# eltoto1219/vltk

Measured on AMD Instinct MI355X. Metric: images/sec FRCNN feature extraction, 800x1333 batch, higher is better.
Workload: dtype f16; 1 GPU; configs[1]: ResNet-101-C4 fp16 (the reference has no FPN: SURVEY.md D1), 32 synthetic 800x1333 images per GPU per step, R=300 RPN proposals through the Res5 head, max 100 detections/img, seeded synthetic weights; global_batch=32, parallelism=image-sharded x1, all-gather of output blocks

## Files before the change

include/vltk_hip.h:

```cpp
#ifndef VLTK_HIP_H
#define VLTK_HIP_H

#include <stddef.h>
#include <stdint.h>

#ifdef __cplusplus
extern "C" {
#endif

#define VK_OK 0
#define VK_EINVAL 1
#define VK_ENOTIMPL 2
#define VK_ENONFINITE 3
#define VK_EWEIGHTS 4
#define VK_EHIP 5
#define VK_ENOMEM 6

typedef enum { VK_F32 = 0, VK_F16 = 1, VK_I64 = 2, VK_I32 = 3, VK_BF16 = 4 } vk_dtype;
typedef enum { VK_ACT_NONE = 0, VK_ACT_RELU = 1, VK_ACT_GELU = 2 , VK_ACT_TANH = 3 } vk_act;

#define VK_MAX_ANCHOR_DIM 8
#define VK_MAX_NMS_THRESH 8

typedef struct vk_config {
// ... 130 lines not shown
int vk_memcpy_d2d(void *dst_dev, const void *src_dev, size_t bytes, void *stream);

int vk_enable_stage_timing(vk_handle *h, int enable);
int vk_get_stage_timing(vk_handle *h, float *ms6);

#define VK_NUM_KERNEL_BUCKETS 12
int vk_enable_kernel_timing(vk_handle *h, int enable);
int vk_get_kernel_timing(vk_handle *h, int64_t *launches, double *ms, double *flops, double *bytes, int reset);


size_t vk_packed_weight_bytes(int cout, int cin, int kh, int kw, int groups, vk_dtype dt);
int vk_packed_cout(int cout);
int vk_conv_slice_channels(int cin, int groups);
int vk_pack_conv_weight(const float *w_oihw_host, const float *bn_host, const float *bias_host,
                        int cout, int cin, int kh, int kw, int groups, vk_dtype dt,
                        void *w_packed_host, float *bias_packed_host);

int vk_conv2d(const void *x, int N, int H, int W, int cin,
              const void *w_packed, const float *bias_packed, const void *residual,
              void *y, int cout, int ldy, int kh, int kw, int stride, int pad, int dil, int groups,
              int relu, vk_dtype dt, vk_dtype out_dt, void *stream);

#define VK_ROUTE_GENERIC 0
#define VK_ROUTE_RING 1
#define VK_ROUTE_DUO 2
#define VK_ROUTE_WS 3
#define VK_ROUTE_GEMM4 4
#define VK_ROUTE_PANEL 5
#define VK_ROUTE_BLK 6
int vk_conv_route(int N, int H, int W, int cin, int cin2, int has_residual, int fused_mean, int cout, int ldy, int kh, int kw,
                  int stride, int pad, int dil, int groups, int relu, vk_dtype dt, vk_dtype out_dt);
int vk_panel_phase_images(int N, int H, int W, int dil);
int vk_panel_phase_tile_rows(int N, int H, int W, int dil, int cout);

int vk_conv1x1_dual(const void *x1, int cin1, const void *x2, int cin2, long M,
                    const void *w_packed, const float *bias_packed, const void *residual,
                    void *y, int cout, int relu, void *stream);

int vk_bottleneck64(const void *x, int N, int H, int W, int cin, int proj,
                    const void *w1_packed, const float *b1_packed, const void *w2_packed, const float *b2_packed,
                    const void *w3_packed, const float *b3_packed, void *y, void *stream);

int vk_fuse_shortcut(int cin, int cin_shortcut, int cout, int stride, vk_dtype dt);
int vk_bottleneck64_eligible(int cin, int cmid, int cout, int stride, int dil, int groups, int proj, int fused_shortcut,
                             long N, int H, int W, vk_dtype dt);

size_t vk_conv1x1_meanpool_workspace_bytes(int N, int HW, int cout);
int vk_conv1x1_meanpool(const void *x, int N, int HW, int cin, const void *w_packed, const float *bias_packed,
                        const void *residual, int cout, int relu, float *out_mean,
                        void *workspace, size_t workspace_bytes, void *stream);


int vk_linear(const void *x, long M, int K, const void *w_packed, const float *bias_packed, const void *residual,
              void *y, int N, int ldy, int act, vk_dtype dt, vk_dtype out_dt, void *stream);
int vk_layernorm(const void *x, int ldx, const float *gamma, const float *beta, void *y, int ldy, int M, int C,
                 float eps, float scale, int accumulate, vk_dtype dt, void *stream);
int vk_embed_layernorm(const int64_t *input_ids, const int64_t *token_type_ids, int B, int L, const void *word,
                       const void *position, const void *token_type, const float *gamma, const float *beta,
                       void *y, int C, float eps, vk_dtype dt, void *stream);
int vk_attention(const void *q, int ldq, const void *k, int ldk, const void *v, int ldv, const float *mask,
                 void *out, int ldo, int B, int heads, int Lq, int Lk, int d, vk_dtype dt, void *stream);
int vk_attention_tiled(const void *q, int ldq, const void *k, int ldk, const void *v, int ldv, const float *mask,
                       void *out, int ldo, int B, int heads, int Lq, int Lk, int d, vk_dtype dt, void *stream);
#define VK_ATT_ROUTE_MFMA 0
#define VK_ATT_ROUTE_LDS 1
#define VK_ATT_ROUTE_TILED 2
// ... 132 lines not shown
```

vltk_amd/_lib.py:

```python
import ctypes as C
import os

_HERE = os.path.dirname(os.path.abspath(__file__))
LIB_PATH = os.path.join(_HERE, "libvltk_hip.so")
if os.environ.get("VLTK_AMD_LIB"):
    LIB_PATH = os.environ["VLTK_AMD_LIB"]
elif os.environ.get("VLTK_AMD_ABLATION_LIB") == "1":
    LIB_PATH = LIB_PATH.replace("libvltk_hip.so", "libvltk_hip_ablation.so")

VK_OK, VK_EINVAL, VK_ENOTIMPL, VK_ENONFINITE, VK_EWEIGHTS, VK_EHIP, VK_ENOMEM = range(7)
VK_F32, VK_F16, VK_I64, VK_I32, VK_BF16 = 0, 1, 2, 3, 4
VK_ACT_NONE, VK_ACT_RELU, VK_ACT_GELU, VK_ACT_TANH = 0, 1, 2, 3
VK_ROUTE_GENERIC, VK_ROUTE_RING, VK_ROUTE_DUO, VK_ROUTE_WS, VK_ROUTE_GEMM4, VK_ROUTE_PANEL, VK_ROUTE_BLK = range(7)
VK_ATT_ROUTE_MFMA, VK_ATT_ROUTE_LDS, VK_ATT_ROUTE_TILED, VK_ATT_ROUTE_STREAM = range(4)
VK_MAX_ANCHOR_DIM = 8
VK_MAX_NMS_THRESH = 8
VK_MAX_IGNOREY = 64
VK_SELECT_CLASS_MAX, VK_SELECT_PER_CLASS, VK_SELECT_DETECTIONS = 0, 1, 2
VK_POOLER_ROIPOOL, VK_POOLER_ROIALIGN, VK_POOLER_ROIALIGNV2 = 0, 1, 2

_EXC = {
    VK_EINVAL: ValueError,
    VK_ENOTIMPL: NotImplementedError,
    VK_ENONFINITE: AssertionError,
# ... 58 lines not shown
    "vk_option_check": (_I, [C.c_char_p, _I]),
    "vk_option_default": (_I, [C.c_char_p, C.POINTER(_I)]),
    "vk_pooler_check": (_I, [_I, _I]),
    "vk_set_pooler": (_I, [_P, _I, _I]),
    "vk_get_pooler": (_I, [_P, C.POINTER(_I), C.POINTER(_I)]),
    "vk_num_weights": (_I, [_P, C.POINTER(_I)]),
    "vk_weight_name": (_I, [_P, _I, C.POINTER(C.c_char_p)]),
    "vk_forward": (_I, [_P, _P, _I, _I, _I, _P, _P, C.POINTER(vk_roi_params), C.POINTER(vk_outputs), _P]),
    "vk_forward_begin": (_I, [_P, _P, _I, _I, _I, _P, _P, C.POINTER(vk_roi_params), C.POINTER(vk_outputs), _P,
                              C.POINTER(C.c_int64)]),
    "vk_forward_begin_ignorey": (_I, [_P, _P, _I, _I, _I, _P, _P, C.POINTER(vk_roi_params), C.POINTER(vk_outputs), _P,
                                      C.POINTER(C.c_int64), C.POINTER(vk_ignorey)]),
    "vk_forward_begin_select": (_I, [_P, _P, _I, _I, _I, _P, _P, C.POINTER(vk_select_params), C.POINTER(vk_outputs), _P,
                                     C.POINTER(C.c_int64), C.POINTER(vk_ignorey)]),
    "vk_forward_boxes_begin": (_I, [_P, _P, _I, _I, _I, _P, _P, _P, _I, _P, C.POINTER(vk_outputs), _P, C.POINTER(C.c_int64)]),
    "vk_forward_grid_begin": (_I, [_P, _P, _I, _I, _I, _P, _P, _I, _I, C.POINTER(vk_outputs), _P, C.POINTER(C.c_int64)]),
    "vk_grid_pool": (_I, [_P, _I, _I, _I, _I, _I, _P, _P, _I, _I, _I, _P, _I, _P, _P]),
    "vk_forward_end": (_I, [_P, C.c_int64]),
    "vk_given_boxes_ingest": (_I, [_P, _P, _P, _P, _I, _I, _P, _P, _P, _I, _I, _F, _I, _P, _P]),
    "vk_given_box_outputs": (_I, [_P, _P, _P, _P, _P, _P, _P, _P, _I, _I, _I, C.POINTER(vk_outputs), _P]),
    "vk_get_stage": (_I, [_P, C.c_char_p, C.POINTER(_P), C.POINTER(_I), C.POINTER(C.c_int64), C.POINTER(_I)]),
    "vk_memcpy_d2d": (_I, [_P, _P, _SZ, _P]),
    "vk_enable_stage_timing": (_I, [_P, _I]),
    "vk_get_stage_timing": (_I, [_P, C.POINTER(_F)]),
    "vk_enable_kernel_timing": (_I, [_P, _I]),
    "vk_get_kernel_timing": (_I, [_P, C.POINTER(C.c_int64), C.POINTER(_D), C.POINTER(_D), C.POINTER(_D), _I]),
    "vk_packed_weight_bytes": (_SZ, [_I, _I, _I, _I, _I, _I]),
    "vk_conv_slice_channels": (_I, [_I, _I]),
    "vk_packed_cout": (_I, [_I]),
    "vk_pack_conv_weight": (_I, [_P, _P, _P, _I, _I, _I, _I, _I, _I, _P, _P]),
    "vk_conv_route": (_I, [_I] * 18),
    "vk_panel_phase_images": (_I, [_I, _I, _I, _I]),
    "vk_panel_phase_tile_rows": (_I, [_I, _I, _I, _I, _I]),
    "vk_conv1x1_dual": (_I, [_P, _I, _P, _I, C.c_long, _P, _P, _P, _P, _I, _I, _P]),
    "vk_bottleneck64": (_I, [_P, _I, _I, _I, _I, _I, _P, _P, _P, _P, _P, _P, _P, _P]),
    "vk_fuse_shortcut": (_I, [_I, _I, _I, _I, _I]),
    "vk_bottleneck64_eligible": (_I, [_I, _I, _I, _I, _I, _I, _I, _I, C.c_long, _I, _I, _I]),
    "vk_conv1x1_meanpool_workspace_bytes": (_SZ, [_I, _I, _I]),
    "vk_conv1x1_meanpool": (_I, [_P, _I, _I, _I, _P, _P, _P, _I, _I, _P, _P, _SZ, _P]),
    "vk_linear": (_I, [_P, C.c_long, _I, _P, _P, _P, _P, _I, _I, _I, _I, _I, _P]),
    "vk_layernorm": (_I, [_P, _I, _P, _P, _P, _I, _I, _I, _F, _F, _I, _I, _P]),
    "vk_embed_layernorm": (_I, [_P, _P, _I, _I, _P, _P, _P, _P, _P, _P, _I, _F, _I, _P]),
    "vk_attention": (_I, [_P, _I, _P, _I, _P, _I, _P, _P, _I, _I, _I, _I, _I, _I, _I, _P]),
    "vk_attention_tiled": (_I, [_P, _I, _P, _I, _P, _I, _P, _P, _I, _I, _I, _I, _I, _I, _I, _P]),
    "vk_attention_route": (_I, [_I] * 9),
    "vk_visualbert_embed": (_I, [_P, _P, _P, _P, _I, _I, _I, _I, _P, _I, _P, _I, _P, _P, _I, _P, _P, _I, _P, _P, _P, _I, _F, _I, _P]),
    "vk_vit_patchify": (_I, [_P, _I, _I, _I, _I, _I, _P, _I, _I, _P]),
    "vk_vit_assemble": (_I, [_P, _I, _P, _P, _I, _I, _P, _I, _I, _P]),
    "vk_roi_align": (_I, [_P, _P, _P, _P, _I, _I, _I, _P, _P, _I, _I, _I, _I, _P, _I, _P]),
    "vk_assign_levels": (_I, [_P, _I, _I, _I, _I, _F, _I, _P, _P]),
    "vk_upsample2x_add": (_I, [_P, _P, _P, _I, _I, _I, _I, _I, _I, _I, _P]),
    "vk_subsample2": (_I, [_P, _P, _I, _I, _I, _I, _I, _P]),
    "vk_relu_copy": (_I, [_P, _P, C.c_long, _I, _P]),
    "vk_rpn_multilevel_workspace_bytes": (_SZ, [_I, _I, _I, _I]),
    "vk_rpn_proposals_multilevel": (_I, [_P, _P, _P, _P, _I, _I, _P, _P, _I, _P, _P, _F, _P, _P, _F, _D, _I, _I, _P, _P, _P, _P, _P, _SZ, _P]),
    "vk_rpn_proposals_multilevel_ignorey": (_I, [_P, _P, _P, _P, _I, _I, _P, _P, _I, _P, _P, _F, _P, _P, _F, _D, _I, _I, _P, _P, _P, _P,
                                                 _P, _SZ, _P, C.POINTER(vk_ignorey)]),
    "vk_conv2d": (_I, [_P, _I, _I, _I, _I, _P, _P, _P, _P, _I, _I, _I, _I, _I, _I, _I, _I, _I, _I, _I, _P]),
    "vk_nchw_to_nhwc": (_I, [_P, _I, _I, _I, _I, _P, _I, _P]),
    "vk_nhwc_to_nchw": (_I, [_P, _I, _I, _I, _I, _P, _I, _P]),
    "vk_packed_stem_bytes": (_SZ, [_I, _I]),
    "vk_pack_stem_weight": (_I, [_P, _P, _I, _I, _P, _P]),
    "vk_stem": (_I, [_P, _I, _I, _I, _P, _P, _I, _I, _P, _I, _P, _SZ, _P]),
    "vk_stem_workspace_bytes": (_SZ, [_I, _I, _I, _I, _I]),
    "vk_stem_out_hw": (None, [_I, _I, _I, C.POINTER(_I), C.POINTER(_I)]),
    "vk_preprocess": (_I, [_P, _P, _P, _I, _I, _I, C.POINTER(_F), C.POINTER(_F), _F, _P, _P]),
# ... 59 lines not shown
```

vltk_amd/csrc/conv3x3_panel.hip:

```cpp
#include <cstdio>
#include <type_traits>
#include <vector>

#include "vk_common.h"

namespace vk {

typedef _Float16 half8 __attribute__((ext_vector_type(8)));
typedef float floatx4 __attribute__((ext_vector_type(4)));
typedef _Float16 half4 __attribute__((ext_vector_type(4)));
typedef unsigned uintx4 __attribute__((ext_vector_type(4)));

struct PanelK {
    const char *x;
    const char *w;
    const float *bias;
    const char *res;
    char *y;
    int H, W, HW, M;
    int cin_bytes, ldy;
    int dil;
    int cstages;
    int wrow_bytes;
    int relu;
// ... 28 lines not shown
constexpr int panel_in_window() {
    int c = 0;
    for (int d = 1; d <= P_NW - 2; ++d) {
        int t = ((J - d) % 9 + 9) % 9;
        if (t < PP) ++c;
    }
    return c;
}
template <int J, int PP, int NWP, bool FIRST>
constexpr int pieces_in_window() {
    static_assert(PP <= 6, "a panel piece of the previous stage in the window of a tap other than 0");
    if (FIRST) return NWP * (P_NW - 2);
    const int c = NWP * (P_NW - 2) + panel_in_window<J, PP>();
    const int after_panel = NWP * (9 - PP);
    return J == 8 && after_panel < c ? after_panel : c;
}
template <int J, int PP, int NWP>
constexpr int last_in_window() {
    int c = 0;
    for (int d = 1; d <= P_NW - 2; ++d) {
        int t = J - d;
        if (t < 0 || t + P_NW < 9) c += NWP;
        if (t < 0 && 9 + t < PP) ++c;
    }
    return c;
}

template <int N>
__device__ __forceinline__ void vm_wait() {
    static_assert(N >= 0 && N <= 15, "vmcnt immediate");
    asm volatile("s_waitcnt vmcnt(%0)" ::"n"(N) : "memory");
}

template <int PP, int DBG, int TAG = 0, int MI = 8, int PHASE = 0, int WR = 2>
__global__ __launch_bounds__(512, 2) void conv3x3_panel_kernel(PanelK p) {
    extern __shared__ __attribute__((aligned(16))) char smem[];
    static_assert(MI == 8 || MI == 9, "8 or 9 row tiles per wave");
    static_assert(WR == 2 || WR == 4, "2 x 4 or 4 x 2 waves");
    static_assert(!PHASE || (PP == (WR == 4 ? 6 : 4) && MI == 8 && !(DBG & 9)), "the phase form: halo 128 = (W / 2 + 1) * 16 at W = 14, 256- or 512-row tiles");
    static_assert(WR == 2 || PHASE == 2, "512 x 128 tiles: the phase form only (a plain res4 launch would read its panel twice)");
    static_assert(MI == 8 || !(DBG & 8), "the LDS-staged epilogue is written for 128-row halves");
    constexpr int WC = 8 / WR;
    constexpr int CT = 64 * WC;
    constexpr int NWP = CT / 128;
    constexpr int WSLOT = CT * 64;
    constexpr int TILE = WR * MI * 16;
    constexpr int PROWS = PP * 128;
    constexpr int HALO = (PROWS - TILE) / 2;
    constexpr int PBYTES = PROWS * 64;
    constexpr int WBASE = 2 * PBYTES;
    static_assert(HALO >= (PHASE ? 128 : 48) && WBASE + P_NW * WSLOT + (PP == 3 || WR == 4 ? 256 : 0) <= 160 * 1024, "halo / LDS");
    constexpr bool ZROW = PP == 3;
    constexpr int ZOFF = WBASE + P_NW * WSLOT;

    int bid = blockIdx.x;
    const int nwg = p.m_tiles * p.n_tiles;
    unsigned long st_k0 = 0;
    if constexpr (DBG & 4) asm volatile("s_memrealtime %0\n\ts_waitcnt lgkmcnt(0)" : "=s"(st_k0)::"memory");
    if constexpr (PP == 3 || PHASE) {
        if (p.tile_ctr && bid >= p.static_tiles) {
            constexpr bool MAIL_IN_PANEL = PHASE && WR == 2;
            int *mail = reinterpret_cast<int *>(smem + (MAIL_IN_PANEL ? 0 : ZOFF + 128));
            if (threadIdx.x == 0) {
                const unsigned v = atomicAdd(p.tile_ctr, 1u);
                if (v == p.ctr_last) *p.tile_ctr = 0u;
                *mail = p.static_tiles + (int)v;
            }
            __syncthreads();
            bid = __builtin_amdgcn_readfirstlane(*mail);
            if constexpr (MAIL_IN_PANEL) __syncthreads();
            if (bid >= nwg) return;
        }
    }
    const int q = nwg >> 3, r = nwg & 7, xcd = bid & 7;
    const int t_ = (xcd < r ? xcd * (q + 1) : r * (q + 1) + (xcd - r) * q) + (bid >> 3);
    const int n_tile = t_ % p.n_tiles, m_tile = t_ / p.n_tiles;
    const int m0 = m_tile * TILE, n0 = n_tile * CT;

    const int tid = threadIdx.x, lane = tid & 63;
    const int wave = __builtin_amdgcn_readfirstlane(tid >> 6);
    const int wr = wave / WC, wc = wave & (WC - 1);
    const int g = lane >> 4, j = lane & 15;

// ... 50 lines not shown
    auto req_w = [&](int slot, int cs, int tap, int i) {
        const unsigned koff = (unsigned)(tap * p.cstages + cs) * 64;
        unsigned wb_ = wsrc0;
        asm volatile("" : "+v"(wb_));
        VKP_GLDS16(p.w + (wb_ + i * wstep + koff), smem + WBASE + slot * WSLOT + (wave * NWP + i) * 1024);
    };

    const unsigned lds0 = (unsigned)(unsigned long)(__attribute__((address_space(3))) char *)smem;
    [[maybe_unused]] const unsigned zrow = lds0 + ZOFF;
    if constexpr (ZROW) {
        if (tid < 16) *reinterpret_cast<unsigned *>(smem + ZOFF + tid * 4) = 0u;
        asm volatile("s_waitcnt lgkmcnt(0)" ::: "memory");
    }
    unsigned w_a[2];
#pragma unroll
    for (int par = 0; par < 2; ++par) {
        const int wrow = wc * 64 + (j >> 2) * 8 + par * 4 + (j & 3);
        w_a[par] = lds0 + WBASE + wrow * 64 + ((g ^ ((-(wrow >> 2)) & 3)) << 4);
    }
    const int jbase = HALO + wr * (MI * 16) + j;
    auto x_addr_of = [&](int parity, int tap) -> unsigned {
        const int shift = PHASE ? ((tap / 3 - 1) * (p.W >> 1) + (tap % 3 - 1)) * 16 : ((tap / 3 - 1) * p.W + (tap % 3 - 1)) * p.dil;
        int jb = jbase;
        asm volatile("" : "+v"(jb));
        const int rb = jb + shift;
        return lds0 + parity * PBYTES + (rb << 6) + ((g ^ ((-(rb >> 2)) & 3)) << 4);
    };

    floatx4 acc[MI][4];
#pragma unroll
    for (int mi = 0; mi < MI; ++mi)
#pragma unroll
        for (int ni = 0; ni < 4; ++ni) acc[mi][ni] = floatx4{0.f, 0.f, 0.f, 0.f};
    half8 wa[4], wb[4], xw[MI == 9 ? 5 : 4];
    const int CS = p.cstages;

#define VKP_DSR(dst, addr, OFF) asm volatile("ds_read_b128 %0, %1 offset:" #OFF : "=v"(dst) : "v"(addr))
#define VKP_DSRX(dst, addr, OFF, TW, J_, MI_)                                                        \
    do {                                                                                             \
        if constexpr (ZROW && !(DBG & 1)) {                                                          \
            unsigned m_, ad_;                                                                        \
            const unsigned zc_ = zrow - (OFF);                                                       \
            asm volatile("v_bfe_i32 %0, %1, %2, 1" : "=v"(m_) : "v"(TW), "n"(((J_) % 3) * 9 + (MI_))); \
            asm volatile("v_bfi_b32 %0, %1, %2, %3" : "=v"(ad_) : "v"(m_), "v"(addr), "s"(zc_));    \
            VKP_DSR(dst, ad_, OFF);                                                                  \
        } else                                                                                       \
            VKP_DSR(dst, addr, OFF);                                                                 \
    } while (0)
#define VKP_WAIT3(reg) asm volatile("s_waitcnt lgkmcnt(3)" : "+v"(reg))
#define VKP_WAIT4(reg) asm volatile("s_waitcnt lgkmcnt(4)" : "+v"(reg))
#define VKP_SB() __builtin_amdgcn_sched_barrier(0)
#define VKP_MMA_ROW(MI, XR, WF, TM)                                                                  \
    do {                                                                                             \
        if constexpr (PHASE == 2) {                                                                  \
            if (((TM) >> (MI)) & 1u) {                           \
                __builtin_amdgcn_s_setprio(1);                                                       \
                _Pragma("unroll") for (int ni = 0; ni < 4; ++ni) acc[MI][ni] =                       \
                    __builtin_amdgcn_mfma_f32_16x16x32_f16(WF[ni], XR, acc[MI][ni], 0, 0, 0);        \
                __builtin_amdgcn_s_setprio(0);                                                       \
            }                                                                                        \
            break;                                                                                   \
        }                                                                                            \
        if constexpr (!(DBG & 1) && !ZROW) {                                                         \
            uintx4 u_ = __builtin_bit_cast(uintx4, XR);                                              \
            const bool v_ = ((TM) >> (MI)) & 1u;                                                     \
            u_[0] = v_ ? u_[0] : 0u;                                                                 \
            u_[1] = v_ ? u_[1] : 0u;                                                                 \
// ... 10 lines not shown
    do {                                                \
        unsigned a0_ = w_a[0], a1_ = w_a[1];            \
        asm volatile("" : "+v"(a0_), "+v"(a1_));        \
        a0_ += so;                                      \
        a1_ += so;                                      \
        VKP_DSR(WF[0], a0_, 0);                         \
        VKP_DSR(WF[1], a1_, 0);                         \
        VKP_DSR(WF[2], a0_, 2048);                      \
        VKP_DSR(WF[3], a1_, 2048);                      \
    } while (0)

    auto tap_mask = [&](auto j_c) -> unsigned {
        constexpr int J = decltype(j_c)::value;
        unsigned tw = J < 3 ? vm0 : (J < 6 ? vm1 : vm2);
        if constexpr (PHASE)
            asm volatile("" : "+s"(tw));
        else
            asm volatile("" : "+v"(tw));
        return tw >> ((J % 3) * 9);
    };
    auto tap_word = [&](auto j_c) -> unsigned {
        constexpr int J = decltype(j_c)::value;
        unsigned tw = J < 3 ? vm0 : (J < 6 ? vm1 : vm2);
        asm volatile("" : "+v"(tw));
        return tw;
    };
    auto pre = [&](auto last_c, auto odd_c, auto j_c, unsigned xa, unsigned &xa_next, const half8 (&wcur)[4], auto first_c) {
        constexpr bool LAST = decltype(last_c)::value, FIRST = decltype(first_c)::value;
        constexpr int ODD = decltype(odd_c)::value;
        constexpr int J = decltype(j_c)::value;
        const unsigned tm = ZROW ? 0u : tap_mask(j_c);
        [[maybe_unused]] const unsigned tw = ZROW ? tap_word(j_c) : 0u;
        constexpr bool has_next = !(LAST && J == 8);
        if constexpr (has_next) xa_next = (J == 8) ? x_addr_of(1 - ODD, 0) : x_addr_of(ODD, J + 1);
        VKP_DSRX(xw[3], xa, 3072, tw, J, 3); VKP_WAIT3(xw[0]); VKP_SB(); VKP_MMA_ROW(0, xw[0], wcur, tm); VKP_SB();
        VKP_DSRX(xw[0], xa, 4096, tw, J, 4); VKP_WAIT3(xw[1]); VKP_SB(); VKP_MMA_ROW(1, xw[1], wcur, tm); VKP_SB();
        VKP_DSRX(xw[1], xa, 5120, tw, J, 5); VKP_WAIT3(xw[2]); VKP_SB(); VKP_MMA_ROW(2, xw[2], wcur, tm); VKP_SB();
        VKP_DSRX(xw[2], xa, 6144, tw, J, 6); VKP_WAIT3(xw[3]); VKP_SB(); VKP_MMA_ROW(3, xw[3], wcur, tm); VKP_SB();
        if constexpr (MI == 9) {
            VKP_DSRX(xw[3], xa, 7168, tw, J, 7); VKP_DSRX(xw[4], xa, 8192, tw, J, 8); VKP_WAIT4(xw[0]); VKP_SB(); VKP_MMA_ROW(4, xw[0], wcur, tm); VKP_SB();
            asm volatile("s_waitcnt lgkmcnt(0)" : "+v"(xw[1]), "+v"(xw[2]), "+v"(xw[3]), "+v"(xw[MI == 9 ? 4 : 3])::"memory");
        } else {
            VKP_DSRX(xw[3], xa, 7168, tw, J, 7); VKP_WAIT3(xw[0]); VKP_SB(); VKP_MMA_ROW(4, xw[0], wcur, tm); VKP_SB();
            asm volatile("s_waitcnt lgkmcnt(0)" : "+v"(xw[1]), "+v"(xw[2]), "+v"(xw[3])::"memory");
        }
        VKP_SB();
        if constexpr (has_next) {
            constexpr int OUT = LAST ? last_in_window<J, PP, NWP>() : pieces_in_window<J, PP, NWP, FIRST>();
            vm_wait<OUT>();
            if constexpr (!(DBG & 48) || ((DBG & 16) && J % 3 == 2)) asm volatile("s_barrier" ::: "memory");
        }
        VKP_SB();
    };
    auto post = [&](auto last_c, auto odd_c, auto j_c, int cs, unsigned xa_next, const half8 (&wcur)[4], half8 (&wnext)[4]) {
        constexpr bool LAST = decltype(last_c)::value;
        constexpr int ODD = decltype(odd_c)::value;
        constexpr int J = decltype(j_c)::value;
        static_assert(!(LAST && J == 8), "the final step has no POST");
        constexpr int SLOT = (3 * ODD + J) % P_NW;
        const unsigned tm = ZROW ? 0u : tap_mask(j_c);
        constexpr int JN = (J + 1) % 9;
        [[maybe_unused]] const unsigned twn = ZROW ? tap_word(std::integral_constant<int, JN>{}) : 0u;
        constexpr bool issue_w = !LAST || (J + P_NW < 9);
        constexpr bool issue_p = !LAST && (J < PP);
        constexpr unsigned so = (unsigned)((SLOT + 1) % P_NW) * WSLOT;
        VKP_READ_W(wnext, so);
        VKP_DSRX(xw[0], xa_next, 0, twn, JN, 0);
        VKP_SB();
        VKP_MMA_ROW(5, xw[1], wcur, tm);
        VKP_SB();
        if constexpr (issue_p) req_panel(cs + 1, J);
        if constexpr (issue_w) req_w(SLOT, cs + (J + P_NW) / 9, (J + P_NW) % 9, 0);
        VKP_DSRX(xw[1], xa_next, 1024, twn, JN, 1);
        VKP_SB();
        VKP_MMA_ROW(6, xw[2], wcur, tm);
        VKP_SB();
        if constexpr (issue_w && NWP == 2) req_w(SLOT, cs + (J + P_NW) / 9, (J + P_NW) % 9, 1);
        VKP_DSRX(xw[2], xa_next, 2048, twn, JN, 2);
        VKP_SB();
        VKP_MMA_ROW(7, xw[3], wcur, tm);
        VKP_SB();
        if constexpr (MI == 9) {
            VKP_MMA_ROW(8, xw[MI == 9 ? 4 : 3], wcur, tm);
            VKP_SB();
        }
    };
    auto wset = [&](auto u_c) -> half8(&)[4] {
        if constexpr (decltype(u_c)::value % 2 == 0)
            return wa;
        else
            return wb;
    };
#define VKP_IC(V) std::integral_constant<int, (V)> {}
#define VKP_UNIT(LP, LC, U)                                                                                          \
    post(LP, VKP_IC(((U) - 1) / 9), VKP_IC(((U) - 1) % 9), cs + ((U) - 1) / 9, xan, wset(VKP_IC((U) - 1)), wset(VKP_IC(U)));  \
    xa = xan;                                                                                                        \
    pre(LC, VKP_IC((U) / 9), VKP_IC((U) % 9), xa, xan, wset(VKP_IC(U)), F_{});
    using T_ = std::integral_constant<bool, true>;
    using F_ = std::integral_constant<bool, false>;

#pragma unroll
    for (int q2 = 0; q2 < PP; ++q2) req_panel(0, q2);
#pragma unroll
    for (int st = 0; st < P_NW; ++st) {
        req_w(st, 0, st, 0);
        if constexpr (NWP == 2) req_w(st, 0, st, 1);
    }
    if constexpr (PHASE) {
        unsigned u0 = 0, u1 = 0, u2 = 0;
#pragma unroll
        for (int mi = 0; mi < MI; ++mi) {
            int G;
            const PhaseBlk b = phase_blk(p, blk_of(wr * MI + mi, G));
// ... 52 lines not shown
            }
        }
    }

    vm_wait<NWP * (P_NW - 1)>();
    asm volatile("s_barrier" ::: "memory");
    unsigned long st_c0 = 0, st_r0 = 0;
    if constexpr (DBG & 4) asm volatile("s_memtime %0\n\ts_memrealtime %1\n\ts_waitcnt lgkmcnt(0)" : "=s"(st_c0), "=s"(st_r0)::"memory");
    unsigned xa = x_addr_of(0, 0), xan = 0;
    VKP_READ_W(wa, 0u);
    {
        [[maybe_unused]] const unsigned tw0 = tap_word(VKP_IC(0));
        VKP_DSRX(xw[0], xa, 0, tw0, 0, 0);
        VKP_DSRX(xw[1], xa, 1024, tw0, 0, 1);
        VKP_DSRX(xw[2], xa, 2048, tw0, 0, 2);
    }
    pre(F_{}, VKP_IC(0), VKP_IC(0), xa, xan, wa, T_{});
    int cs = 0;
    for (; cs + 2 < CS; cs += 2) {
        VKP_UNIT(F_{}, F_{}, 1) VKP_UNIT(F_{}, F_{}, 2) VKP_UNIT(F_{}, F_{}, 3) VKP_UNIT(F_{}, F_{}, 4) VKP_UNIT(F_{}, F_{}, 5)
        VKP_UNIT(F_{}, F_{}, 6) VKP_UNIT(F_{}, F_{}, 7) VKP_UNIT(F_{}, F_{}, 8) VKP_UNIT(F_{}, F_{}, 9) VKP_UNIT(F_{}, F_{}, 10)
        VKP_UNIT(F_{}, F_{}, 11) VKP_UNIT(F_{}, F_{}, 12) VKP_UNIT(F_{}, F_{}, 13) VKP_UNIT(F_{}, F_{}, 14) VKP_UNIT(F_{}, F_{}, 15)
        VKP_UNIT(F_{}, F_{}, 16) VKP_UNIT(F_{}, F_{}, 17)
        post(F_{}, VKP_IC(1), VKP_IC(8), cs + 1, xan, wb, wa);
        xa = xan;
        pre(F_{}, VKP_IC(0), VKP_IC(0), xa, xan, wa, F_{});
    }
    VKP_UNIT(F_{}, F_{}, 1) VKP_UNIT(F_{}, F_{}, 2) VKP_UNIT(F_{}, F_{}, 3) VKP_UNIT(F_{}, F_{}, 4) VKP_UNIT(F_{}, F_{}, 5)
    VKP_UNIT(F_{}, F_{}, 6) VKP_UNIT(F_{}, F_{}, 7) VKP_UNIT(F_{}, F_{}, 8) VKP_UNIT(F_{}, T_{}, 9) VKP_UNIT(T_{}, T_{}, 10)
    VKP_UNIT(T_{}, T_{}, 11) VKP_UNIT(T_{}, T_{}, 12) VKP_UNIT(T_{}, T_{}, 13) VKP_UNIT(T_{}, T_{}, 14) VKP_UNIT(T_{}, T_{}, 15)
    VKP_UNIT(T_{}, T_{}, 16) VKP_UNIT(T_{}, T_{}, 17)
    {
        const unsigned tm = ZROW ? 0u : tap_mask(VKP_IC(8));
        VKP_MMA_ROW(5, xw[1], wb, tm);
        VKP_MMA_ROW(6, xw[2], wb, tm);
        VKP_MMA_ROW(7, xw[3], wb, tm);
        if constexpr (MI == 9) VKP_MMA_ROW(8, xw[MI == 9 ? 4 : 3], wb, tm);
    }
    unsigned long st_c1 = 0, st_r1 = 0;
    if constexpr (DBG & 4) asm volatile("s_memtime %0\n\ts_memrealtime %1\n\ts_waitcnt lgkmcnt(0)" : "=s"(st_c1), "=s"(st_r1)::"memory");
#undef VKP_UNIT
#undef VKP_IC
#undef VKP_DSR
#undef VKP_DSRX
#undef VKP_WAIT3
#undef VKP_WAIT4
#undef VKP_MMA_ROW
#undef VKP_READ_W
#undef VKP_SB

    if constexpr (!(DBG & 8)) {
        if constexpr (PHASE) asm volatile("" : "+s"(g0), "+s"(gb0));
        auto epilogue = [&](auto res_c, auto relu_c, auto full_c) {
            constexpr bool RES = decltype(res_c)::value, RELU = decltype(relu_c)::value, FULL = decltype(full_c)::value;
            const int ch0 = n0 + wc * 64 + g * 8;
            floatx4 bq[2][2];
#pragma unroll
            for (int qn = 0; qn < 2; ++qn) {
                bq[qn][0] = *reinterpret_cast<const floatx4 *>(p.bias + ch0 + qn * 32);
                bq[qn][1] = *reinterpret_cast<const floatx4 *>(p.bias + ch0 + qn * 32 + 4);
            }
#pragma unroll
            for (int mi = 0; mi < MI; ++mi) {
                const long m = m0 + wr * (MI * 16) + mi * 16 + j;
                long mo = m;
                if constexpr (PHASE) {
                    int G;
                    const int t = blk_of(wr * MI + mi, G);
                    mo = (long)(G * 16 + j) * p.HW + phase_blk(p, t).row;
// ... 125 lines not shown
    if (panel_pp(a, 9) == 0) return 8;
    if (const char *v = getenv("VK_PANEL_MI")) {
        if (v[0] == '8') return 8;
        if (v[0] == '9') return 9;
    }
    const long nt = a.Cout / 256;
    const long n8 = ((M + 255) / 256 * nt + n_cu - 1) / n_cu, n9 = ((M + 287) / 288 * nt + n_cu - 1) / n_cu;
    if (n8 > 4) return 9;
    return n9 * 9 < n8 * 8 ? 9 : 8;
}

bool conv3x3_panel_eligible(const ConvArgs &a) {
    const char *v = getenv("VK_CONV3X3_PANEL");
    if (v && v[0] == '0') return false;
    if (a.stem || a.dt != VK_F16 || a.out_dt != VK_F16 || a.relu > 1) return false;
    if (a.kh != 3 || a.kw != 3 || a.stride != 1 || a.pad != a.dil) return false;
    if (a.Cout % 256 != 0 || a.ldy != a.Cout || a.Cin % 64 != 0 || a.Cin < 128) return false;
    if (panel_pp(a) == 0) return false;
    if ((long)a.N * a.H * a.W * a.Cin * 2 >= (1L << 32)) return false;
    return true;
}

int conv3x3_panel_phase_images(const ConvArgs &a) {
    const char *v = getenv("VK_PANEL_PHASE");
    if (v && v[0] == '0') return 0;
    if (a.dil != 2 || a.H % 2 != 0 || a.W % 2 != 0 || a.W > 14 || a.H > 1024 || a.N < 16) return 0;
    return a.N / 16 * 16;
}

int conv3x3_panel_phase_tile_rows(const ConvArgs &a) {
    if (a.Cout % 256 != 0 || conv3x3_panel_phase_images(a) == 0) return 0;
    const char *v = getenv("VK_PANEL_TALL");
    return v && v[0] == '0' ? 256 : 512;
}

static int launch_panel_one(const ConvArgs &a, hipStream_t stream, bool phase);

int launch_conv3x3_panel(const ConvArgs &a, hipStream_t stream) {
    const int np = conv3x3_panel_phase_images(a);
    if (np == 0) return launch_panel_one(a, stream, false);
    ConvArgs b = a;
    b.N = np;
    VK_TRY(launch_panel_one(b, stream, true));
    if (np == a.N) return VK_OK;
    const size_t rows = (size_t)np * a.H * a.W;
    b.N = a.N - np;
    b.x = (const char *)a.x + rows * a.Cin * 2;
    b.y = (char *)a.y + rows * a.ldy * 2;
    if (a.res) b.res = (const char *)a.res + rows * a.ldy * 2;
    return launch_panel_one(b, stream, false);
}

static int launch_panel_one(const ConvArgs &a, hipStream_t stream, bool phase) {
    DeviceState *ds = nullptr;
    VK_TRY(device_state(&ds));
    PanelK k;
    k.x = (const char *)a.x;
    k.w = (const char *)a.w;
    k.bias = a.bias;
    k.res = (const char *)a.res;
    k.y = (char *)a.y;
    k.H = a.H;
    k.W = a.W;
    k.HW = a.H * a.W;
    const long M = (long)a.N * a.H * a.W;
    VK_REQUIRE(M > 0 && M < (1L << 31) - 512, VK_EINVAL, "conv3x3_panel: M=%ld out of range", M);
// ... 49 lines not shown
        if (mi == 9)
            VKP_LAUNCH(3, 4, 0, 9);
        else
            VKP_LAUNCH(3, 4, 0, 8);
        VK_CHECK_HIP(hipStreamSynchronize(stream));
        std::vector<unsigned long> h((size_t)grid.x * 6);
        VK_CHECK_HIP(hipMemcpy(h.data(), k.stamps, nb, hipMemcpyDeviceToHost));
        VK_CHECK_HIP(hipFree(k.stamps));
        if (FILE *f = fopen(sf, "a")) {
            fprintf(f, "# wg k_loop_cycles k_loop_ticks workgroup_ticks ticks_before_k_loop start_tick end_tick (tick = 10 ns)\n");
            for (unsigned w = 0; w < grid.x; ++w)
                fprintf(f, "%u %lu %lu %lu %lu %lu %lu\n", w, h[(size_t)w * 6], h[(size_t)w * 6 + 1], h[(size_t)w * 6 + 2], h[(size_t)w * 6 + 3], h[(size_t)w * 6 + 4],
                        h[(size_t)w * 6 + 5]);
            fclose(f);
        }
    } else if (mi == 8 && pp == 3 && dbg == 8)
        VKP_LAUNCH(3, 8, 0, 8);
    else if (mi == 8 && pp == 3 && dbg == 1)
        VKP_LAUNCH(3, 1, 0, 8);
    else if (mi == 9 && pp == 3 && dbg == 1)
        VKP_LAUNCH(3, 1, 0, 9);
    else if (mi == 9 && pp == 3 && dbg == 16)
        VKP_LAUNCH(3, 16, 0, 9);
    else if (mi == 9 && pp == 3 && dbg == 32)
        VKP_LAUNCH(3, 32, 0, 9);
    else
#endif
#ifdef VK_ABLATION
    if (const char *pv = getenv("VK_PANEL_PHASE"); phase && pv && pv[0] == 'A') {
        VK_TRY(set_max_lds(conv3x3_panel_kernel<4, 0, 0, 8, 1>, smem));
        hipLaunchKernelGGL((conv3x3_panel_kernel<4, 0, 0, 8, 1>), grid, block, smem, stream, k);
    } else
#endif
    if (tall) {
        VK_TRY(set_max_lds(conv3x3_panel_kernel<6, 0, 0, 8, 2, 4>, smem));
        hipLaunchKernelGGL((conv3x3_panel_kernel<6, 0, 0, 8, 2, 4>), grid, block, smem, stream, k);
    } else if (phase) {
        VK_TRY(set_max_lds(conv3x3_panel_kernel<4, 0, 0, 8, 2>, smem));
        hipLaunchKernelGGL((conv3x3_panel_kernel<4, 0, 0, 8, 2>), grid, block, smem, stream, k);
    } else if (mi == 8 && pp == 3 && a.concurrent)
        VKP_LAUNCH(3, 0, 1, 8);
    else if (mi == 8 && pp == 3)
        VKP_LAUNCH(3, 0, 0, 8);
    else if (mi == 8 && a.concurrent)
        VKP_LAUNCH(4, 0, 1, 8);
    else if (mi == 8)
        VKP_LAUNCH(4, 0, 0, 8);
    else if (pp == 3 && a.concurrent)
        VKP_LAUNCH(3, 0, 1, 9);
    else if (pp == 3)
        VKP_LAUNCH(3, 0, 0, 9);
    else if (a.concurrent)
        VKP_LAUNCH(4, 0, 1, 9);
    else
        VKP_LAUNCH(4, 0, 0, 9);
#undef VKP_LAUNCH
    VK_CHECK_HIP(hipGetLastError());
    return t.end(stream, a.concurrent ? 6 : 4, 2.0 * (double)k.M * a.Cout * 9 * a.Cin, k.M, a.Cout, a.Cin, 9, 1,
                 2.0 * ((double)k.M * a.Cin + (double)k.M * a.Cout * (a.res ? 2 : 1) + (double)a.Cout * 9 * a.Cin));
}

}
```

vltk_amd/csrc/stage_api.hip:

```cpp
#include <algorithm>
#include <cmath>
#include <cstdlib>

#include "vk_common.h"

using namespace vk;

namespace vk {

void fill_conv_args(ConvArgs &a, int N, int H, int W, int cin, int cout, int ldy, int k, int stride, int pad, int dil, int groups,
                    int relu, vk_dtype dt, vk_dtype out_dt) {
    memset(&a, 0, sizeof(a));
    a.N = N;
    a.H = H;
    a.W = W;
    a.Cin = cin;
    conv_out_hw(H, W, k, stride, pad, dil, &a.Ho, &a.Wo);
    a.Cout = cout;
    a.ldy = ldy;
    a.kh = a.kw = k;
    a.stride = stride;
    a.pad = pad;
    a.dil = dil;
    a.groups = groups;
// ... 157 lines not shown
int vk_conv_route(int N, int H, int W, int cin, int cin2, int has_residual, int fused_mean, int cout, int ldy, int kh, int kw,
                  int stride, int pad, int dil, int groups, int relu, vk_dtype dt, vk_dtype out_dt) {
    if (!(kh == kw && kh >= 1 && stride >= 1 && dil >= 1 && pad >= 0 && groups >= 1 && cin2 >= 0)) {
        set_error("conv_route: bad geometry");
        return -VK_EINVAL;
    }
    static const char here = 0;
    ConvArgs a;
    fill_conv_args(a, N, H, W, cin, cout, ldy, kh, stride, pad, dil, groups, relu, dt, out_dt);
    if (!(a.Ho > 0 && a.Wo > 0 && N > 0)) {
        set_error("conv_route: empty output");
        return -VK_EINVAL;
    }
    a.x = a.w = &here;
    a.res = has_residual ? &here : nullptr;
    a.x2 = cin2 > 0 ? &here : nullptr;
    a.Cin2 = cin2;
    a.pool_part = fused_mean ? (float *)&here : nullptr;
    return conv_route_checked(a);
}

int vk_panel_phase_images(int N, int H, int W, int dil) {
    ConvArgs a;
    fill_conv_args(a, N, H, W, 128, 256, 256, 3, 1, dil, dil, 1, 0, VK_F16, VK_F16);
    return conv3x3_panel_phase_images(a);
}

int vk_panel_phase_tile_rows(int N, int H, int W, int dil, int cout) {
    ConvArgs a;
    fill_conv_args(a, N, H, W, 128, cout, cout, 3, 1, dil, dil, 1, 0, VK_F16, VK_F16);
    return conv3x3_panel_phase_tile_rows(a);
}

int vk_conv1x1_dual(const void *x1, int cin1, const void *x2, int cin2, long M, const void *w_packed, const float *bias_packed,
                    const void *residual, void *y, int cout, int relu, void *stream) {
    VK_REQUIRE(x1 && x2 && M > 0 && M < (1L << 31), VK_EINVAL, "conv1x1_dual: bad arguments");
    ConvArgs a;
    fill_conv_args(a, 1, 1, (int)M, cin1, cout, cout, 1, 1, 0, 1, 1, relu, VK_F16, VK_F16);
    a.x = x1;
    a.x2 = x2;
    a.Cin2 = cin2;
    a.w = w_packed;
    a.bias = bias_packed;
    a.res = residual;
    a.y = y;
    return launch_conv(a, (hipStream_t)stream);
}

int vk_conv1x1_rows(const void *x1, int cin1, const void *x2, int cin2, long M, const int32_t *m_dev, const int32_t *x2_idx,
                    const void *w_packed, const float *bias_packed, void *y, int cout, int relu, void *stream) {
    VK_REQUIRE(x1 && w_packed && bias_packed && y && M > 0 && M < (1L << 31), VK_EINVAL, "conv1x1_rows: bad arguments");
    VK_REQUIRE(!x2_idx || x2, VK_EINVAL, "conv1x1_rows: a row index needs a second input");
    ConvArgs a;
    fill_conv_args(a, 1, 1, (int)M, cin1, cout, cout, 1, 1, 0, 1, 1, relu, VK_F16, VK_F16);
    a.x = x1;
    a.x2 = x2;
    a.Cin2 = x2 ? cin2 : 0;
    a.w = w_packed;
    a.bias = bias_packed;
    a.y = y;
    VK_REQUIRE(conv_route(a) == VK_ROUTE_GEMM4, VK_EINVAL, "conv1x1_rows: the layer does not run as VK_ROUTE_GEMM4 at %ld rows", M);
    a.m_dev = m_dev;
    a.x2_idx = x2_idx;
    return launch_conv_gemm4(a, (hipStream_t)stream);
}

// ... 231 lines not shown
```

vltk_amd/csrc/vk_common.h:

```cpp
#pragma once
#include <hip/hip_runtime.h>

#include <atomic>
#include <cstdarg>
#include <cstdint>
#include <cstdio>
#include <cstring>
#include <vector>

#include "vltk_hip.h"

namespace vk {

void set_error(const char *fmt, ...);

#define VK_CHECK_HIP(expr)                                                                    \
    do {                                                                                      \
        hipError_t _e = (expr);                                                               \
        if (_e != hipSuccess) {                                                               \
            vk::set_error("%s:%d: %s -> %s", __FILE__, __LINE__, #expr, hipGetErrorString(_e)); \
            return VK_EHIP;                                                                   \
        }                                                                                     \
    } while (0)

// ... 30 lines not shown
constexpr int CONV_BM = 128;
constexpr int CONV_KTILE_BYTES = 128;
constexpr int CONV_COUT_ALIGN = 128;

struct ConvArgs {
    const void *x;
    const void *w;
    const float *bias;
    const void *res;
    void *y;
    int N, H, W, Cin;
    int Ho, Wo, Cout, ldy;
    int kh, kw, stride, pad, dil;
    int groups;
    int concurrent;
    float *pool_part;
    const void *x2;
    int Cin2;
    int relu;
    int stem;
    const int32_t *m_dev;
    const int32_t *x2_idx;
    vk_dtype dt, out_dt;
};
int launch_conv(const ConvArgs &a, hipStream_t stream);
int conv_route(const ConvArgs &a);
int conv_route_checked(const ConvArgs &a);
bool conv256_eligible(const ConvArgs &a);
int launch_conv256(const ConvArgs &a, hipStream_t stream);
bool conv3x3_panel_eligible(const ConvArgs &a);
int launch_conv3x3_panel(const ConvArgs &a, hipStream_t stream);
int conv3x3_panel_phase_images(const ConvArgs &a);
int conv3x3_panel_phase_tile_rows(const ConvArgs &a);
bool conv_gemm4_eligible(const ConvArgs &a);
int launch_conv_gemm4(const ConvArgs &a, hipStream_t stream);
int acquire_tile_counter(unsigned **ctr);
bool conv256_dual_ok(const ConvArgs &a);
bool conv_duo_eligible(const ConvArgs &a);
int launch_conv_duo(const ConvArgs &a, hipStream_t stream);
bool conv_ws_eligible(const ConvArgs &a);
int launch_conv_ws(const ConvArgs &a, hipStream_t stream);
bool conv3x3_blk_eligible(const ConvArgs &a);
int launch_conv3x3_blk(const ConvArgs &a, hipStream_t stream);
bool bneck_fused_eligible(int cin, int cmid, int cout, int stride, int groups, bool proj, long N, int H, int W, vk_dtype dt);
int launch_bneck_fused(const void *x, int N, int H, int W, int cin, bool proj, const void *w1, const float *b1, const void *w2,
                       const float *b2, const void *w3, const float *b3, void *y, bool concurrent, hipStream_t stream);
bool conv_duo_dual_ok(const ConvArgs &a);
bool conv_duo_pool_ok(const ConvArgs &a);
size_t conv_duo_pool_part_bytes(long M, int Cout);
bool conv_pool_sums_f64(long N, int HW, int Cin, int Cout, bool dual);
bool conv_ws_pool_ok(const ConvArgs &a);
int launch_pool_finish(const float *part, int N, int HoWo, int Cin, int Cout, bool dual, float *out, hipStream_t stream);

struct KernelTimer {
    struct Rec {
        int bucket;
        double flops;
        hipEvent_t e0, e1;
        int M, cout, cin, k, stride;
        double bytes;
    };
    std::vector<Rec> recs;
    std::vector<hipEvent_t> pool;
    std::vector<hipEvent_t> all;
    int64_t launches[VK_NUM_KERNEL_BUCKETS] = {};
    double ms[VK_NUM_KERNEL_BUCKETS] = {};
// ... 200 lines not shown
```

Measured before the change: 524.8 images/sec.

## Reuse input fragments across horizontal taps in tall panel 3x3 conv

Adds a REUSE variant of the 512x128 phase panel conv kernel. It keeps a 10-slot register window of input fragments, so the three horizontal taps (dx = -1, 0, +1) share loaded 16-row tiles, and each later tap issues only one new LDS read instead of eight. This cuts LDS read traffic and waits in the MFMA inner loop, at the cost of more VGPRs (10 fragments instead of 4) and a changed overlap schedule. The variant is on by default for 512-row tiles and can be switched off with VK_PANEL_REUSE=0.

```diff
diff --git a/include/vltk_hip.h b/include/vltk_hip.h
--- a/include/vltk_hip.h
+++ b/include/vltk_hip.h
@@ -186,6 +186,7 @@
                   int stride, int pad, int dil, int groups, int relu, vk_dtype dt, vk_dtype out_dt);
 int vk_panel_phase_images(int N, int H, int W, int dil);
 int vk_panel_phase_tile_rows(int N, int H, int W, int dil, int cout);
+int vk_panel_phase_reuse(int N, int H, int W, int dil, int cout);
 
 int vk_conv1x1_dual(const void *x1, int cin1, const void *x2, int cin2, long M,
                     const void *w_packed, const float *bias_packed, const void *residual,
diff --git a/vltk_amd/_lib.py b/vltk_amd/_lib.py
--- a/vltk_amd/_lib.py
+++ b/vltk_amd/_lib.py
@@ -114,6 +114,7 @@
     "vk_conv_route": (_I, [_I] * 18),
     "vk_panel_phase_images": (_I, [_I, _I, _I, _I]),
     "vk_panel_phase_tile_rows": (_I, [_I, _I, _I, _I, _I]),
+    "vk_panel_phase_reuse": (_I, [_I, _I, _I, _I, _I]),
     "vk_conv1x1_dual": (_I, [_P, _I, _P, _I, C.c_long, _P, _P, _P, _P, _I, _I, _P]),
     "vk_bottleneck64": (_I, [_P, _I, _I, _I, _I, _I, _P, _P, _P, _P, _P, _P, _P, _P]),
     "vk_fuse_shortcut": (_I, [_I, _I, _I, _I, _I]),
diff --git a/vltk_amd/csrc/conv3x3_panel.hip b/vltk_amd/csrc/conv3x3_panel.hip
--- a/vltk_amd/csrc/conv3x3_panel.hip
+++ b/vltk_amd/csrc/conv3x3_panel.hip
@@ -84,7 +84,26 @@
     asm volatile("s_waitcnt vmcnt(%0)" ::"n"(N) : "memory");
 }
 
-template <int PP, int DBG, int TAG = 0, int MI = 8, int PHASE = 0, int WR = 2>
+constexpr int P_WIN = 10;
+constexpr int reuse_slot(int dx, int mi) { return mi + dx + 1; }
+constexpr int reuse_tile(int dy, int slot, int w2) { return dy * w2 + slot - 1; }
+constexpr int reuse_read_dx(int slot) { return slot < 8 ? -1 : slot - 8; }
+constexpr bool reuse_window_ok() {
+    for (int w2 = 1; w2 <= 7; ++w2)
+        for (int dy = -1; dy <= 1; ++dy)
+            for (int dx = -1; dx <= 1; ++dx)
+                for (int mi = 0; mi < 8; ++mi) {
+                    const int s = reuse_slot(dx, mi);
+                    if (s < 0 || s >= P_WIN) return false;
+                    if (reuse_tile(dy, s, w2) != mi + dy * w2 + dx) return false;
+                    if (reuse_read_dx(s) > dx) return false;
+                    if (reuse_tile(dy, s, w2) < -8 || reuse_tile(dy, s, w2) > 15) return false;
+                }
+    return true;
+}
+static_assert(reuse_window_ok(), "REUSE: (tap, row tile) -> window slot -> panel tile, W / 2 = 1 .. 7, inside tiles b - 8 .. b + 15");
+
+template <int PP, int DBG, int TAG = 0, int MI = 8, int PHASE = 0, int WR = 2, int REUSE = 0>
 __global__ __launch_bounds__(512, 2) void conv3x3_panel_kernel(PanelK p) {
     extern __shared__ __attribute__((aligned(16))) char smem[];
     static_assert(MI == 8 || MI == 9, "8 or 9 row tiles per wave");
@@ -92,6 +111,7 @@
     static_assert(!PHASE || (PP == (WR == 4 ? 6 : 4) && MI == 8 && !(DBG & 9)), "the phase form: halo 128 = (W / 2 + 1) * 16 at W = 14, 256- or 512-row tiles");
     static_assert(WR == 2 || PHASE == 2, "512 x 128 tiles: the phase form only (a plain res4 launch would read its panel twice)");
     static_assert(MI == 8 || !(DBG & 8), "the LDS-staged epilogue is written for 128-row halves");
+    static_assert(!REUSE || (PHASE == 2 && WR == 4 && MI == 8 && DBG == 0), "the fragment window: tap shifts of whole 16-row tiles, 512 x 128 tiles");
     constexpr int WC = 8 / WR;
     constexpr int CT = 64 * WC;
     constexpr int NWP = CT / 128;
@@ -101,6 +121,7 @@
     constexpr int HALO = (PROWS - TILE) / 2;
     constexpr int PBYTES = PROWS * 64;
     constexpr int WBASE = 2 * PBYTES;
+    static_assert(!REUSE || (HALO / 16 == 8 && HALO / 16 + (WR - 1) * MI + 15 < PROWS / 16), "REUSE: the halo (8 tiles) covers tiles b - 8 .. b + 15");
     static_assert(HALO >= (PHASE ? 128 : 48) && WBASE + P_NW * WSLOT + (PP == 3 || WR == 4 ? 256 : 0) <= 160 * 1024, "halo / LDS");
     constexpr bool ZROW = PP == 3;
     constexpr int ZOFF = WBASE + P_NW * WSLOT;
@@ -217,7 +238,7 @@
     for (int mi = 0; mi < MI; ++mi)
 #pragma unroll
         for (int ni = 0; ni < 4; ++ni) acc[mi][ni] = floatx4{0.f, 0.f, 0.f, 0.f};
-    half8 wa[4], wb[4], xw[MI == 9 ? 5 : 4];
+    half8 wa[4], wb[4], xw[REUSE ? P_WIN : (MI == 9 ? 5 : 4)];
     const int CS = p.cstages;
 
 #define VKP_DSR(dst, addr, OFF) asm volatile("ds_read_b128 %0, %1 offset:" #OFF : "=v"(dst) : "v"(addr))
@@ -294,17 +315,46 @@
         const unsigned tm = ZROW ? 0u : tap_mask(j_c);
         [[maybe_unused]] const unsigned tw = ZROW ? tap_word(j_c) : 0u;
         constexpr bool has_next = !(LAST && J == 8);
-        if constexpr (has_next) xa_next = (J == 8) ? x_addr_of(1 - ODD, 0) : x_addr_of(ODD, J + 1);
-        VKP_DSRX(xw[3], xa, 3072, tw, J, 3); VKP_WAIT3(xw[0]); VKP_SB(); VKP_MMA_ROW(0, xw[0], wcur, tm); VKP_SB();
-        VKP_DSRX(xw[0], xa, 4096, tw, J, 4); VKP_WAIT3(xw[1]); VKP_SB(); VKP_MMA_ROW(1, xw[1], wcur, tm); VKP_SB();
-        VKP_DSRX(xw[1], xa, 5120, tw, J, 5); VKP_WAIT3(xw[2]); VKP_SB(); VKP_MMA_ROW(2, xw[2], wcur, tm); VKP_SB();
-        VKP_DSRX(xw[2], xa, 6144, tw, J, 6); VKP_WAIT3(xw[3]); VKP_SB(); VKP_MMA_ROW(3, xw[3], wcur, tm); VKP_SB();
-        if constexpr (MI == 9) {
-            VKP_DSRX(xw[3], xa, 7168, tw, J, 7); VKP_DSRX(xw[4], xa, 8192, tw, J, 8); VKP_WAIT4(xw[0]); VKP_SB(); VKP_MMA_ROW(4, xw[0], wcur, tm); VKP_SB();
-            asm volatile("s_waitcnt lgkmcnt(0)" : "+v"(xw[1]), "+v"(xw[2]), "+v"(xw[3]), "+v"(xw[MI == 9 ? 4 : 3])::"memory");
+        if constexpr (REUSE) {
+            constexpr int D = J % 3;
+            if constexpr (has_next && D == 2)
+                xa_next = (J == 8) ? x_addr_of(1 - ODD, 0) : x_addr_of(ODD, J + 1);
+            else
+                xa_next = xa;
+#define VKP_ROWX(MI_) VKP_SB(); VKP_MMA_ROW(MI_, xw[reuse_slot(D - 1, MI_)], wcur, tm); VKP_SB()
+            if constexpr (D == 0) {
+                static_assert(reuse_slot(-1, 4) == 4 && reuse_read_dx(7) == -1);
+                VKP_DSR(xw[3], xa, 3072); VKP_WAIT3(xw[0]); VKP_ROWX(0);
+                VKP_DSR(xw[4], xa, 4096); VKP_WAIT3(xw[1]); VKP_ROWX(1);
+                VKP_DSR(xw[5], xa, 5120); VKP_WAIT3(xw[2]); VKP_ROWX(2);
+                VKP_DSR(xw[6], xa, 6144); VKP_WAIT3(xw[3]); VKP_ROWX(3);
+                VKP_DSR(xw[7], xa, 7168); VKP_WAIT3(xw[4]); VKP_ROWX(4);
+                asm volatile("s_waitcnt lgkmcnt(0)" : "+v"(xw[5]), "+v"(xw[6]), "+v"(xw[7])::"memory");
+            } else {
+                static_assert(reuse_read_dx(7 + D) == D - 1 && reuse_slot(D - 1, 7) == 7 + D);
+                half8(&wm)[4] = (9 * ODD + J) % 2 == 0 ? wa : wb;
+                asm volatile("s_waitcnt lgkmcnt(0)" : "+v"(wm[0]), "+v"(wm[1]), "+v"(wm[2]), "+v"(wm[3]));
+                if constexpr (D == 1)
+                    VKP_DSR(xw[8], xa, 8192);
+                else
+                    VKP_DSR(xw[9], xa, 9216);
+                VKP_ROWX(0); VKP_ROWX(1); VKP_ROWX(2); VKP_ROWX(3); VKP_ROWX(4);
+                asm volatile("s_waitcnt lgkmcnt(0)" : "+v"(xw[7 + D])::"memory");
+            }
+#undef VKP_ROWX
         } else {
-            VKP_DSRX(xw[3], xa, 7168, tw, J, 7); VKP_WAIT3(xw[0]); VKP_SB(); VKP_MMA_ROW(4, xw[0], wcur, tm); VKP_SB();
-            asm volatile("s_waitcnt lgkmcnt(0)" : "+v"(xw[1]), "+v"(xw[2]), "+v"(xw[3])::"memory");
+            if constexpr (has_next) xa_next = (J == 8) ? x_addr_of(1 - ODD, 0) : x_addr_of(ODD, J + 1);
+            VKP_DSRX(xw[3], xa, 3072, tw, J, 3); VKP_WAIT3(xw[0]); VKP_SB(); VKP_MMA_ROW(0, xw[0], wcur, tm); VKP_SB();
+            VKP_DSRX(xw[0], xa, 4096, tw, J, 4); VKP_WAIT3(xw[1]); VKP_SB(); VKP_MMA_ROW(1, xw[1], wcur, tm); VKP_SB();
+            VKP_DSRX(xw[1], xa, 5120, tw, J, 5); VKP_WAIT3(xw[2]); VKP_SB(); VKP_MMA_ROW(2, xw[2], wcur, tm); VKP_SB();
+            VKP_DSRX(xw[2], xa, 6144, tw, J, 6); VKP_WAIT3(xw[3]); VKP_SB(); VKP_MMA_ROW(3, xw[3], wcur, tm); VKP_SB();
+            if constexpr (MI == 9) {
+                VKP_DSRX(xw[3], xa, 7168, tw, J, 7); VKP_DSRX(xw[4], xa, 8192, tw, J, 8); VKP_WAIT4(xw[0]); VKP_SB(); VKP_MMA_ROW(4, xw[0], wcur, tm); VKP_SB();
+                asm volatile("s_waitcnt lgkmcnt(0)" : "+v"(xw[1]), "+v"(xw[2]), "+v"(xw[3]), "+v"(xw[MI == 9 ? 4 : 3])::"memory");
+            } else {
+                VKP_DSRX(xw[3], xa, 7168, tw, J, 7); VKP_WAIT3(xw[0]); VKP_SB(); VKP_MMA_ROW(4, xw[0], wcur, tm); VKP_SB();
+                asm volatile("s_waitcnt lgkmcnt(0)" : "+v"(xw[1]), "+v"(xw[2]), "+v"(xw[3])::"memory");
+            }
         }
         VKP_SB();
         if constexpr (has_next) {
@@ -326,21 +376,24 @@
         constexpr bool issue_w = !LAST || (J + P_NW < 9);
         constexpr bool issue_p = !LAST && (J < PP);
         constexpr unsigned so = (unsigned)((SLOT + 1) % P_NW) * WSLOT;
+        constexpr int D = J % 3;
+        constexpr bool ahead = !REUSE || D == 2;
+        constexpr int X5 = REUSE ? reuse_slot(D - 1, 5) : 1, X6 = REUSE ? reuse_slot(D - 1, 6) : 2, X7 = REUSE ? reuse_slot(D - 1, 7) : 3;
         VKP_READ_W(wnext, so);
-        VKP_DSRX(xw[0], xa_next, 0, twn, JN, 0);
+        if constexpr (ahead) VKP_DSRX(xw[0], xa_next, 0, twn, JN, 0);
         VKP_SB();
-        VKP_MMA_ROW(5, xw[1], wcur, tm);
+        VKP_MMA_ROW(5, xw[X5], wcur, tm);
         VKP_SB();
         if constexpr (issue_p) req_panel(cs + 1, J);
         if constexpr (issue_w) req_w(SLOT, cs + (J + P_NW) / 9, (J + P_NW) % 9, 0);
-        VKP_DSRX(xw[1], xa_next, 1024, twn, JN, 1);
+        if constexpr (ahead) VKP_DSRX(xw[1], xa_next, 1024, twn, JN, 1);
         VKP_SB();
-        VKP_MMA_ROW(6, xw[2], wcur, tm);
+        VKP_MMA_ROW(6, xw[X6], wcur, tm);
         VKP_SB();
         if constexpr (issue_w && NWP == 2) req_w(SLOT, cs + (J + P_NW) / 9, (J + P_NW) % 9, 1);
-        VKP_DSRX(xw[2], xa_next, 2048, twn, JN, 2);
+        if constexpr (ahead) VKP_DSRX(xw[2], xa_next, 2048, twn, JN, 2);
         VKP_SB();
-        VKP_MMA_ROW(7, xw[3], wcur, tm);
+        VKP_MMA_ROW(7, xw[X7], wcur, tm);
         VKP_SB();
         if constexpr (MI == 9) {
             VKP_MMA_ROW(8, xw[MI == 9 ? 4 : 3], wcur, tm);
@@ -459,9 +512,9 @@
     VKP_UNIT(T_{}, T_{}, 16) VKP_UNIT(T_{}, T_{}, 17)
     {
         const unsigned tm = ZROW ? 0u : tap_mask(VKP_IC(8));
-        VKP_MMA_ROW(5, xw[1], wb, tm);
-        VKP_MMA_ROW(6, xw[2], wb, tm);
-        VKP_MMA_ROW(7, xw[3], wb, tm);
+        VKP_MMA_ROW(5, xw[REUSE ? reuse_slot(1, 5) : 1], wb, tm);
+        VKP_MMA_ROW(6, xw[REUSE ? reuse_slot(1, 6) : 2], wb, tm);
+        VKP_MMA_ROW(7, xw[REUSE ? reuse_slot(1, 7) : 3], wb, tm);
         if constexpr (MI == 9) VKP_MMA_ROW(8, xw[MI == 9 ? 4 : 3], wb, tm);
     }
     unsigned long st_c1 = 0, st_r1 = 0;
@@ -653,6 +706,12 @@
     if (a.Cout % 256 != 0 || conv3x3_panel_phase_images(a) == 0) return 0;
     const char *v = getenv("VK_PANEL_TALL");
     return v && v[0] == '0' ? 256 : 512;
+}
+
+int conv3x3_panel_phase_reuse(const ConvArgs &a) {
+    if (conv3x3_panel_phase_tile_rows(a) != 512) return 0;
+    const char *v = getenv("VK_PANEL_REUSE");
+    return v && v[0] == '0' ? 0 : 1;
 }
 
 static int launch_panel_one(const ConvArgs &a, hipStream_t stream, bool phase);
@@ -768,7 +827,10 @@
         hipLaunchKernelGGL((conv3x3_panel_kernel<4, 0, 0, 8, 1>), grid, block, smem, stream, k);
     } else
 #endif
-    if (tall) {
+    if (tall && conv3x3_panel_phase_reuse(a)) {
+        VK_TRY(set_max_lds(conv3x3_panel_kernel<6, 0, 0, 8, 2, 4, 1>, smem));
+        hipLaunchKernelGGL((conv3x3_panel_kernel<6, 0, 0, 8, 2, 4, 1>), grid, block, smem, stream, k);
+    } else if (tall) {
         VK_TRY(set_max_lds(conv3x3_panel_kernel<6, 0, 0, 8, 2, 4>, smem));
         hipLaunchKernelGGL((conv3x3_panel_kernel<6, 0, 0, 8, 2, 4>), grid, block, smem, stream, k);
     } else if (phase) {
diff --git a/vltk_amd/csrc/stage_api.hip b/vltk_amd/csrc/stage_api.hip
--- a/vltk_amd/csrc/stage_api.hip
+++ b/vltk_amd/csrc/stage_api.hip
@@ -213,6 +213,12 @@
     return conv3x3_panel_phase_tile_rows(a);
 }
 
+int vk_panel_phase_reuse(int N, int H, int W, int dil, int cout) {
+    ConvArgs a;
+    fill_conv_args(a, N, H, W, 128, cout, cout, 3, 1, dil, dil, 1, 0, VK_F16, VK_F16);
+    return conv3x3_panel_phase_reuse(a);
+}
+
 int vk_conv1x1_dual(const void *x1, int cin1, const void *x2, int cin2, long M, const void *w_packed, const float *bias_packed,
                     const void *residual, void *y, int cout, int relu, void *stream) {
     VK_REQUIRE(x1 && x2 && M > 0 && M < (1L << 31), VK_EINVAL, "conv1x1_dual: bad arguments");
diff --git a/vltk_amd/csrc/vk_common.h b/vltk_amd/csrc/vk_common.h
--- a/vltk_amd/csrc/vk_common.h
+++ b/vltk_amd/csrc/vk_common.h
@@ -86,6 +86,7 @@
 int launch_conv3x3_panel(const ConvArgs &a, hipStream_t stream);
 int conv3x3_panel_phase_images(const ConvArgs &a);
 int conv3x3_panel_phase_tile_rows(const ConvArgs &a);
+int conv3x3_panel_phase_reuse(const ConvArgs &a);
 bool conv_gemm4_eligible(const ConvArgs &a);
 int launch_conv_gemm4(const ConvArgs &a, hipStream_t stream);
 int acquire_tile_counter(unsigned **ctr);
```

After: 531.5 images/sec (median of 6 runs). +1.3%, better.
